# powturbo/Turbo-Range-Coder

Hardware: AMD Instinct MI355X
Metric: encode+decode MB/s, order-0 static-CDF rANS, 100 MB bytes (higher is better)
Workload: dtype u32; 1 GPU; text100m: 100000000 B/GPU, static-CDF rANS, 2 states (anscdf4senc/anscdf4sdec per chunk), tables in LDS, chunk 512 B, 1 lane = 1 chunk, 64 chunks/wave; codec=anscdf4s, chunk=512, bytes_per_gpu=100000000, compressed_bytes_per_gpu=64522350, steps_in_flight=1, exchange=none

## Files before the change

turbo-range-coder_amd/csrc/trc_dir.hip:

```cpp
#include <stdlib.h>
#include "trc_dev.h"
#include "trc_launch.h"

__global__ __launch_bounds__(256) void trc_static_prep_kernel(const u16 *__restrict__ cdf, u32 cdfnum,
                                                              u8 *__restrict__ tables)
{
    __shared__ u32 c[258];
    const u32 tid = threadIdx.x;
    for (u32 i = tid; i < 258; i += 256) c[i] = (i <= cdfnum) ? (u32)cdf[i] : TRC_PROB_ONE;
    __syncthreads();
    const u32 slot = blockIdx.x * 256 + tid;
    u32 x = 0, hi = 256;
    while (x + 1 < hi) { u32 mid = (x + hi) >> 1; if (c[mid] > slot) hi = mid; else x = mid; }
    tables[TRC_TAB_LUT + slot] = (u8)x;
    if (blockIdx.x == 0) {
        const u32 c0 = c[tid], f = c[tid + 1] - c0;
        uint4 e; u32 d;
        if (f == 0) {
            e = make_uint4(0u, 0u, 0xffffffffu, 0u); d = 1u << 16;
        } else if (f == 1) {
            e = make_uint4(0xffffffffu, TRC_PROB_ONE - 1u, 1u << 16, c0 + TRC_PROB_ONE - 1u); d = (1u << 16) | c0;
        } else {
            const u32 l = 32u - (u32)__clz((int)(f - 1));
            const u32 m = (u32)((((u64)1) << (31 + l)) / f) + 1u;
            e = make_uint4(m, (TRC_PROB_ONE - f) | ((l - 1u) << 24), f << 16, c0);
            d = (f << 16) | c0;
        }
        ((uint4 *)(tables + TRC_TAB_ENC))[tid] = e;
        ((u32 *)(tables + TRC_TAB_DEC))[tid] = d;
        for (u32 i = tid; i < 260; i += 256) ((u16 *)(tables + TRC_TAB_CDF))[i] = (u16)((i <= cdfnum) ? cdf[i] : TRC_PROB_ONE);
    }
}

void trc_launch_static_prep(const uint16_t *d_cdf, unsigned cdfnum, uint8_t *tables, hipStream_t s)
{
    hipLaunchKernelGGL(trc_static_prep_kernel, dim3(128), dim3(256), 0, s, d_cdf, (u32)cdfnum, tables);
}

__global__ __launch_bounds__(256) void trc_group_sums_kernel(const u32 *__restrict__ clen, u32 nchunks, u64 n, u32 chunk,
                                                             u32 *__restrict__ gsum)
{
    const u32 c = blockIdx.x * 256 + threadIdx.x;
    const u64 cstart = (u64)c * chunk;
    const u32 len = c < nchunks ? (u32)((n - cstart) < chunk ? (n - cstart) : chunk) : 0u;
    const u32 v = trc_wave_sum(c < nchunks ? trc_min(clen[c], len) : 0u);
    if (trc_lane() == 0 && (c >> 6) < ((nchunks + 63) >> 6)) gsum[c >> 6] = v;
}
void trc_launch_group_sums(const uint32_t *d_clen, uint32_t nchunks, size_t n, uint32_t chunk, uint32_t *gsum, hipStream_t s)
{
    hipLaunchKernelGGL(trc_group_sums_kernel, dim3((nchunks + 255) / 256), dim3(256), 0, s, d_clen, nchunks, (u64)n, chunk, gsum);
}

__global__ __launch_bounds__(1024) void trc_scan_groups_kernel(const u32 *__restrict__ gsum, u32 ngroups,
                                                               u64 *__restrict__ goff, u64 *__restrict__ total)
{
    __shared__ u32 wsum[16];
    __shared__ u64 base_s;
    const u32 tid = threadIdx.x, lane = tid & 63, wid = tid >> 6;
    if (tid == 0) base_s = 0;
    __syncthreads();
    for (u32 t0 = 0; t0 < ngroups; t0 += 1024) {
        const u32 i = t0 + tid;
        const u32 v = i < ngroups ? gsum[i] : 0u;
        const u32 inc = trc_wave_incl_scan(v);
        if (lane == 63) wsum[wid] = inc;
        __syncthreads();
        u32 wbase = 0;
        for (u32 k = 0; k < wid; k++) wbase += wsum[k];
        const u64 base = base_s;
        if (i < ngroups) goff[i] = base + wbase + inc - v;
        __syncthreads();
        if (tid == 1023) base_s = base + wbase + inc;
        __syncthreads();
    }
    if (tid == 0) { goff[ngroups] = base_s; if (total) *total = base_s; }
}
void trc_launch_scan_groups(const uint32_t *gsum, uint32_t ngroups, uint64_t *goff, uint64_t *d_total, hipStream_t s)
{
    TRC_LAUNCH_TIMED(trc_scan_groups_kernel, dim3(1), dim3(1024), 0, s, gsum, ngroups, goff, d_total);
}

__global__ __launch_bounds__(256) void trc_range_dir_kernel(const u32 *__restrict__ clen, u32 nchunks, u64 n, u32 chunk,
                                                            const u64 *__restrict__ goff_full, u32 first, u32 count,
                                                            u32 *__restrict__ gsum_sub, u64 *__restrict__ goff_sub)
{
    const u32 ngroups_sub = (count + 63u) >> 6, end = first + count;
    const u32 j = blockIdx.x * 4u + (threadIdx.x >> 6), lane = trc_lane();
    if (j > ngroups_sub) return;
    const u32 b = trc_min(first + 64u * j, end);
    auto clamped = [&](u32 c) -> u32 {
        const u64 left = n - (u64)c * chunk;
        return trc_min(clen[c], left < chunk ? (u32)left : chunk);
    };
    const u32 below = (b & ~63u) + lane, mine = b + lane;
    const u32 pre = trc_wave_sum(below < b ? clamped(below) : 0u);
    const u32 sum = trc_wave_sum(mine < end ? clamped(mine) : 0u);
    if (lane == 0) {
        goff_sub[j] = goff_full[b >> 6] + pre;
        if (j < ngroups_sub) gsum_sub[j] = sum;
    }
}
void trc_launch_range_dir(const uint32_t *d_clen, uint32_t nchunks, size_t n, uint32_t chunk, const uint64_t *goff_full,
                          uint32_t first, uint32_t count, uint32_t *gsum_sub, uint64_t *goff_sub, hipStream_t s)
{
    const uint32_t waves = (count + 63u) / 64u + 1u;
    hipLaunchKernelGGL(trc_range_dir_kernel, dim3((waves + 3u) / 4u), dim3(256), 0, s, d_clen, nchunks, (u64)n, chunk, goff_full,
                       first, count, gsum_sub, goff_sub);
}

#ifndef TRC_GATHER_VPT
#define TRC_GATHER_VPT 6
#endif
#ifndef TRC_GATHER_ATTR
#define TRC_GATHER_ATTR
#endif
template <int PARTS>
__global__ __launch_bounds__(256) TRC_GATHER_ATTR void trc_gather_kernel(const u8 *__restrict__ in, u64 n, u32 chunk, u32 nchunks,
                                                         const u8 *__restrict__ scratch, u32 stride, int from_end,
                                                         const u8 *__restrict__ scratch2, u32 stride2, const u32 *__restrict__ aux,
                                                         const u32 *__restrict__ clen, const u64 *__restrict__ goff,
                                                         const u32 *__restrict__ gsum, u32 ngroups,
                                                         u8 *__restrict__ payload, u64 *__restrict__ total, u64 *__restrict__ goff_out)
{
    constexpr u32 NP = 64u * PARTS;
    constexpr u32 TPP = 256u / NP;
    constexpr u32 VPT = TRC_GATHER_VPT;
    __shared__ u32 ex_s[NP + 1];
    __shared__ u64 src_s[NP];
    __shared__ u64 base_s;
    const u32 g = blockIdx.x, tid = threadIdx.x, lane = tid & 63u, wid = tid >> 6;
    if (wid == 1 || blockDim.x == 64) {
        const u64 b = trc_group_base(goff, gsum, g);
        if (lane == 0) { base_s = b; if (goff_out) goff_out[g] = b; }
    }
    if (wid == 0) {
        const u32 c = g * 64 + lane;
        const u32 l = c < nchunks ? clen[c] : 0u;
        const u64 cstart = (u64)c * chunk;
        const u32 len = c < nchunks ? (u32)((n - cstart) < chunk ? (n - cstart) : chunk) : 0u;
        const bool raw = l == len;
        const u32 inc = trc_wave_incl_scan(l);
        if (PARTS == 1) {
            ex_s[lane] = inc - l;
            src_s[lane] = (u64)(uintptr_t)(raw ? in + cstart : from_end ? scratch + (u64)(c + 1) * stride - l : scratch + (u64)c * stride);
        } else {
            const u8 *a = scratch + (u64)c * stride;
            const u32 la = (raw || c >= nchunks) ? l : from_end >= 3 ? aux[2 * c] : 4u + *(const u32 *)a;
            ex_s[2 * lane] = inc - l; ex_s[2 * lane + 1] = inc - l + la;
            src_s[2 * lane] = (u64)(uintptr_t)(raw ? in + cstart : from_end == 4 ? scratch + (u64)(c + 1) * stride - la : a);
            src_s[2 * lane + 1] = (u64)(uintptr_t)(from_end == 3 ? scratch + (u64)(c + 1) * stride - (l - la) :
                                                   from_end == 4 ? scratch2 + (u64)(c + 1) * stride2 - (l - la) : scratch2 + (u64)c * stride2);
        }
        if (lane == 63) ex_s[NP] = inc;
    }
    __syncthreads();
    const u64 base = base_s;
    const u32 tot = ex_s[NP];
    if (total && g == ngroups - 1 && tid == 0) *total = base + tot;
    u8 *dst0 = payload + base;
    auto src_of = [&](u32 p) -> const u8 * { return (const u8 *)(uintptr_t)src_s[p]; };

    u32 head = (u32)((16u - ((uintptr_t)dst0 & 15u)) & 15u);
    if (head > tot) head = tot;
    const u32 nvec = (tot - head) >> 4;
    const u32 tail0 = head + (nvec << 4);
    for (u32 b = tid; b < head + (tot - tail0); b += 256) {
        const u32 d = b < head ? b : tail0 + (b - head);
        u32 lo = 0, hi = NP;
        while (lo + 1 < hi) { const u32 mid = (lo + hi) >> 1; if (ex_s[mid] <= d) lo = mid; else hi = mid; }
        dst0[d] = src_of(lo)[d - ex_s[lo]];
    }
    {
        const u32 k = tid / TPP, sub = tid % TPP;
        const u32 e0 = ex_s[k], e1 = ex_s[k + 1];
        const u32 v_lo = e0 <= head ? 0u : (e0 - head + 15u) >> 4;
        u32 v_hi = e1 <= head ? 0u : (e1 - head + 15u) >> 4;
        if (v_hi > nvec) v_hi = nvec;
        const u8 *sa = src_of(k);
        const u8 *sb = k + 1 < NP ? src_of(k + 1) : sa;
        const u32 e2 = ex_s[k + 2 > NP ? NP : k + 2];
        const u32 pl = e1 - e0;
        const bool a16 = pl >= 16u;
        const bool b16 = k + 1 < NP && e2 - e1 >= 16u;
        auto bytewise = [&](u32 dv) {
            u32 kk = k;
            const u8 *p = sa;
            for (u32 q = 0; q < 16; q++) {
                while (dv + q >= ex_s[kk + 1]) { kk++; p = src_of(kk); }
                dst0[dv + q] = p[dv + q - ex_s[kk]];
            }
        };
        if (!a16) {
            if (sub == 0 && v_lo < v_hi) bytewise(head + (v_lo << 4));
            return;
        }
        for (u32 v0 = v_lo + sub; v0 < v_hi; v0 += VPT * TPP) {
            uint4 a[VPT], b[VPT];
            u32 d[VPT];
            bool ok[VPT];
#pragma unroll
            for (int j = 0; j < (int)VPT; j++) {
                const u32 v = v0 + TPP * (u32)j;
                ok[j] = v < v_hi;
                d[j] = head + ((ok[j] ? v : v0) << 4);
                a[j] = make_uint4(0u, 0u, 0u, 0u);
                if (ok[j]) a[j] = trc_ld16_a2_global(sa + trc_min(d[j] - e0, pl - 16u));
                b[j] = a[j];
            }
#pragma unroll
            for (int j = 0; j < (int)VPT; j++)
                if (ok[j] && d[j] + 16u > e1 && b16) b[j] = trc_ld16_a2_global(sb);
#pragma unroll
            for (int j = 0; j < (int)VPT; j++) {
                if (!ok[j]) continue;
                const u32 sp = e1 - d[j];
                if (sp >= 16u) { *(uint4 *)(dst0 + d[j]) = a[j]; continue; }
                if (b16) *(uint4 *)(dst0 + d[j]) = trc_splice16(a[j], b[j], 16u - sp);
                else bytewise(d[j]);
            }
        }
    }
}
void trc_launch_gather(const uint8_t *d_in, size_t n, uint32_t chunk, const TrcWork &w, TrcGather mode,
                       const uint32_t *d_clen, uint8_t *d_payload, uint64_t *d_total, hipStream_t s)
{
    const int from_end = mode;
    if (from_end >= 2)
        TRC_LAUNCH_TIMED((trc_gather_kernel<2>), dim3(w.ngroups), dim3(256), 0, s, d_in, (u64)n, chunk, w.nchunks,
                           w.scratch, w.stride, from_end >= 3 ? from_end : 0, w.scratch2, w.stride2, w.aux, d_clen, w.goff, w.gsum, w.ngroups,
                           d_payload, w.goff ? (u64 *)nullptr : d_total, w.goff ? (u64 *)nullptr : w.goff_area);
    else
        TRC_LAUNCH_TIMED((trc_gather_kernel<1>), dim3(w.ngroups), dim3(256), 0, s, d_in, (u64)n, chunk, w.nchunks,
                           w.scratch, w.stride, from_end, w.scratch2, w.stride2, w.aux, d_clen, w.goff, w.gsum, w.ngroups,
                           d_payload, w.goff ? (u64 *)nullptr : d_total, w.goff ? (u64 *)nullptr : w.goff_area);
}

#define TRC_HIST2_WAVE_LDS (128u * 16u * 4u)
#define TRC_HIST2_WAVES 16u
#define TRC_HIST2_ROUND_VECS 1023u
__global__ __launch_bounds__(1024) void trc_hist2_kernel(const u8 *__restrict__ in, u64 n, u64 *__restrict__ hist, u32 round_vecs)
{
    extern __shared__ __attribute__((aligned(16))) u8 smem[];
    typedef __attribute__((address_space(3))) u32 lds_u32;
    const u32 tid = threadIdx.x, lane = tid & 63u, wv = tid >> 6;
    u32 *mine = (u32 *)(smem + wv * TRC_HIST2_WAVE_LDS);
    u64 *tot = (u64 *)(smem + TRC_HIST2_WAVES * TRC_HIST2_WAVE_LDS);
    const u32 col = trc_lds_addr(mine) + (lane & 15u) * 4u;
    if (tid < 256u) tot[tid] = 0;
    const u64 nvec = n >> 4, stride = (u64)gridDim.x * 1024;
    const uint4 *v = (const uint4 *)in;
    auto count = [&](u32 w) __attribute__((always_inline)) {
#pragma unroll
        for (int k = 0; k < 4; k++) {
            const u32 a = (__builtin_amdgcn_ubfe(w, 8 * k + 1, 7) << 6) + col;
            const u32 inc = __umul24(__builtin_amdgcn_ubfe(w, 8 * k, 1), 0xffffu) + 1u;
            __hip_atomic_fetch_add((lds_u32 *)(uintptr_t)a, inc, __ATOMIC_RELAXED, __HIP_MEMORY_SCOPE_WAVEFRONT);
        }
    };
    auto count4 = [&](const uint4 q) __attribute__((always_inline)) { count(q.x); count(q.y); count(q.z); count(q.w); };
    for (u64 r0 = 0; r0 == 0 || r0 < nvec; r0 += stride * round_vecs) {
        for (u32 r = lane; r < 128u * 16u; r += 64u) mine[r] = 0;
        u64 i = r0 + (u64)blockIdx.x * 1024 + tid;
        u32 left = round_vecs;
        if (left >= 2u && i + stride < nvec) {
            uint4 q0 = v[i], q1 = v[i + stride];
            left -= 2u; i += 2 * stride;
            for (; left >= 2u && i + stride < nvec; left -= 2u, i += 2 * stride) {
                const uint4 n0 = v[i], n1 = v[i + stride];
                count4(q0); count4(q1);
                q0 = n0; q1 = n1;
            }
            count4(q0); count4(q1);
        }
        for (; left && i < nvec; left--, i += stride) count4(v[i]);
        if (r0 == 0 && blockIdx.x == 0 && wv == 0)
            for (u64 t = (nvec << 4) + lane; t < n; t += 64) {
                const u32 b = in[t];
                __hip_atomic_fetch_add((lds_u32 *)(uintptr_t)(col + (b >> 1) * 64u), (b & 1u) ? 0x10000u : 1u, __ATOMIC_RELAXED, __HIP_MEMORY_SCOPE_WAVEFRONT);
            }
        u32 lo0 = 0, hi0 = 0, lo1 = 0, hi1 = 0;
#pragma unroll
        for (u32 c4 = 0; c4 < 4u; c4++) {
            const uint4 a = *(const uint4 *)(mine + lane * 16u + c4 * 4u), b = *(const uint4 *)(mine + (lane + 64u) * 16u + c4 * 4u);
            lo0 += (a.x & 0xffffu) + (a.y & 0xffffu) + (a.z & 0xffffu) + (a.w & 0xffffu); hi0 += (a.x >> 16) + (a.y >> 16) + (a.z >> 16) + (a.w >> 16);
            lo1 += (b.x & 0xffffu) + (b.y & 0xffffu) + (b.z & 0xffffu) + (b.w & 0xffffu); hi1 += (b.x >> 16) + (b.y >> 16) + (b.z >> 16) + (b.w >> 16);
        }
        __syncthreads();
        atomicAdd((unsigned long long *)&tot[2 * lane], (unsigned long long)lo0);
        atomicAdd((unsigned long long *)&tot[2 * lane + 1], (unsigned long long)hi0);
        atomicAdd((unsigned long long *)&tot[2 * (lane + 64)], (unsigned long long)lo1);
        atomicAdd((unsigned long long *)&tot[2 * (lane + 64) + 1], (unsigned long long)hi1);
    }
    __syncthreads();
    if (tid < 256u) {
        const u32 bin = (tid + 37u * blockIdx.x) & 255u;
        if (tot[bin]) atomicAdd((unsigned long long *)&hist[bin], (unsigned long long)tot[bin]);
    }
}
__global__ __launch_bounds__(256) void trc_cdf_build_kernel(const u64 *__restrict__ hist, u64 n, u32 cdfnum,
                                                            u16 *__restrict__ cdf, int *__restrict__ status)
{
    __shared__ u64 f[256];
    __shared__ u32 pre[257];
    __shared__ int bad;
    const u32 tid = threadIdx.x;
    if (tid == 0) bad = 0;
    u64 v = 0;
    if (tid < cdfnum) { v = (hist[tid] << TRC_PROB_BITS) / n; if (!v) v = 1; }
    f[tid] = v;
    __syncthreads();
    if (tid == 0) {
        u64 best = 0, sum = 0; u32 bi = 0;
        for (u32 i = 0; i < cdfnum; i++) { sum += f[i]; if (f[i] > best) { best = f[i]; bi = i; } }
        f[bi] -= sum - TRC_PROB_ONE;
        u32 acc = 0; pre[0] = 0;
        for (u32 i = 0; i < cdfnum; i++) { acc = (acc + (u32)f[i]) & 0xffffu; pre[i + 1] = acc; }
    }
    __syncthreads();
    if (tid < cdfnum && pre[tid] >= pre[tid + 1]) atomicOr(&bad, 1);
    if (tid == 0 && pre[cdfnum] != (TRC_PROB_ONE & 0xffffu)) atomicOr(&bad, 1);
    __syncthreads();
    for (u32 i = tid; i <= cdfnum; i += 256) cdf[i] = (u16)pre[i];
    if (tid == 0) *status = bad ? -1 : (int)(n > 0x7fffffffull ? 0x7fffffffull : n);
}
void trc_launch_hist(const uint8_t *d_in, size_t n, uint64_t *d_hist, hipStream_t s)
{
    (void)hipMemsetAsync(d_hist, 0, 256 * sizeof(uint64_t), s);
    const size_t sm2 = TRC_HIST2_WAVES * TRC_HIST2_WAVE_LDS + 256u * sizeof(u64);
    u64 b2 = ((n >> 4) + 1023) / 1024;
    b2 = b2 < 1 ? 1 : b2 > 256 ? 256 : b2;
    TRC_RAISE_LDS_ONCE(trc_hist2_kernel, sm2);
    static const u32 rv = getenv("TRC_HIST_ROUND_VECS") ? (u32)atoi(getenv("TRC_HIST_ROUND_VECS")) : TRC_HIST2_ROUND_VECS;
    hipLaunchKernelGGL(trc_hist2_kernel, dim3((u32)b2), dim3(1024), sm2, s, d_in, (u64)n, d_hist,
                       rv >= 1u && rv <= TRC_HIST2_ROUND_VECS ? rv : TRC_HIST2_ROUND_VECS);
}
void trc_launch_cdf_build(const uint64_t *d_hist, size_t n_total, uint16_t *d_cdf, unsigned cdfnum, int32_t *d_status, hipStream_t s)
{
    hipLaunchKernelGGL(trc_cdf_build_kernel, dim3(1), dim3(256), 0, s, d_hist, (u64)n_total, (u32)cdfnum, d_cdf, d_status);
}
void trc_launch_cdfini(const uint8_t *d_in, size_t n, uint16_t *d_cdf, unsigned cdfnum,
                       int32_t *d_status, uint64_t *d_hist, hipStream_t s)
{
    trc_launch_hist(d_in, n, d_hist, s);
    trc_launch_cdf_build(d_hist, n, d_cdf, cdfnum, d_status, s);
}
```

Baseline: 729,500 MB/s.

## Restructure gather into 64-byte-aligned sectors with per-piece ownership and edge vectors

Result: faster. 739,300 MB/s (median of 6 runs) (+1.3%).

```diff
diff --git a/turbo-range-coder_amd/csrc/trc_dir.hip b/turbo-range-coder_amd/csrc/trc_dir.hip
--- a/turbo-range-coder_amd/csrc/trc_dir.hip
+++ b/turbo-range-coder_amd/csrc/trc_dir.hip
@@ -114,6 +114,9 @@
 #ifndef TRC_GATHER_ATTR
 #define TRC_GATHER_ATTR
 #endif
+#ifdef TRC_GATHER_PROF
+__device__ unsigned long long trc_gat_wall[16 * 4096];
+#endif
 template <int PARTS>
 __global__ __launch_bounds__(256) TRC_GATHER_ATTR void trc_gather_kernel(const u8 *__restrict__ in, u64 n, u32 chunk, u32 nchunks,
                                                          const u8 *__restrict__ scratch, u32 stride, int from_end,
@@ -129,6 +132,9 @@
     __shared__ u64 src_s[NP];
     __shared__ u64 base_s;
     const u32 g = blockIdx.x, tid = threadIdx.x, lane = tid & 63u, wid = tid >> 6;
+#ifdef TRC_GATHER_PROF
+    const u64 gw0 = wall_clock64();
+#endif
     if (wid == 1 || blockDim.x == 64) {
         const u64 b = trc_group_base(goff, gsum, g);
         if (lane == 0) { base_s = b; if (goff_out) goff_out[g] = b; }
@@ -154,6 +160,9 @@
         if (lane == 63) ex_s[NP] = inc;
     }
     __syncthreads();
+#ifdef TRC_GATHER_PROF
+    const u64 gw1 = wall_clock64();
+#endif
     const u64 base = base_s;
     const u32 tot = ex_s[NP];
     if (total && g == ngroups - 1 && tid == 0) *total = base + tot;
@@ -164,63 +173,116 @@
     if (head > tot) head = tot;
     const u32 nvec = (tot - head) >> 4;
     const u32 tail0 = head + (nvec << 4);
+    const u32 sh = (u32)((64u - ((uintptr_t)dst0 & 63u)) & 63u);
+    const u32 nsec = tot > sh ? (tot - sh) >> 6 : 0u;
+    auto bytewise = [&](u32 dv, u32 kk) {
+        const u8 *p = src_of(kk);
+        for (u32 q = 0; q < 16; q++) {
+            while (dv + q >= ex_s[kk + 1]) { kk++; p = src_of(kk); }
+            dst0[dv + q] = p[dv + q - ex_s[kk]];
+        }
+    };
+    auto piece_of = [&](u32 d) -> u32 {
+        u32 lo = 0, hi = NP;
+        while (lo + 1 < hi) { const u32 mid = (lo + hi) >> 1; if (ex_s[mid] <= d) lo = mid; else hi = mid; }
+        return lo;
+    };
     for (u32 b = tid; b < head + (tot - tail0); b += 256) {
         const u32 d = b < head ? b : tail0 + (b - head);
-        u32 lo = 0, hi = NP;
-        while (lo + 1 < hi) { const u32 mid = (lo + hi) >> 1; if (ex_s[mid] <= d) lo = mid; else hi = mid; }
+        const u32 lo = piece_of(d);
         dst0[d] = src_of(lo)[d - ex_s[lo]];
+    }
+    {
+        const u32 nv1 = ((tot < sh ? tot : sh) - head) >> 4;
+        const u32 nv2 = nvec - nv1 - 4u * nsec;
+        const u32 e = tid - 64u;
+        if (e < nv1 + nv2) {
+            const u32 dv = e < nv1 ? head + (e << 4) : sh + (nsec << 6) + ((e - nv1) << 4);
+            const u32 lo = piece_of(dv);
+            if (dv + 16u <= ex_s[lo + 1]) *(uint4 *)(dst0 + dv) = trc_ld16_a2_global(src_of(lo) + (dv - ex_s[lo]));
+            else bytewise(dv, lo);
+        }
     }
     {
         const u32 k = tid / TPP, sub = tid % TPP;
         const u32 e0 = ex_s[k], e1 = ex_s[k + 1];
-        const u32 v_lo = e0 <= head ? 0u : (e0 - head + 15u) >> 4;
-        u32 v_hi = e1 <= head ? 0u : (e1 - head + 15u) >> 4;
-        if (v_hi > nvec) v_hi = nvec;
-        const u8 *sa = src_of(k);
-        const u8 *sb = k + 1 < NP ? src_of(k + 1) : sa;
-        const u32 e2 = ex_s[k + 2 > NP ? NP : k + 2];
-        const u32 pl = e1 - e0;
-        const bool a16 = pl >= 16u;
-        const bool b16 = k + 1 < NP && e2 - e1 >= 16u;
-        auto bytewise = [&](u32 dv) {
-            u32 kk = k;
-            const u8 *p = sa;
-            for (u32 q = 0; q < 16; q++) {
-                while (dv + q >= ex_s[kk + 1]) { kk++; p = src_of(kk); }
-                dst0[dv + q] = p[dv + q - ex_s[kk]];
+        const u32 s_lo = e0 <= sh ? 0u : (e0 - sh + 63u) >> 6;
+        u32 s_hi = e1 <= sh ? 0u : (e1 - sh + 63u) >> 6;
+        if (s_hi > nsec) s_hi = nsec;
+        if (s_lo < s_hi) {
+            const u8 *sa = src_of(k);
+            const u8 *sb = k + 1 < NP ? src_of(k + 1) : sa;
+            const u32 e2 = ex_s[k + 2 > NP ? NP : k + 2];
+            const u32 pl = e1 - e0;
+            const bool a16 = pl >= 16u;
+            const bool b16 = k + 1 < NP && e2 - e1 >= 16u;
+            constexpr u32 LV = 4u / TPP;
+            enum { WHOLE, SPLICE, BYTES };
+            uint4 la[LV], lb[LV];
+            u32 ld[LV], lk[LV];
+#pragma unroll
+            for (int i = 0; i < (int)LV; i++) {
+                const u32 d = sh + ((4u * (s_hi - 1u) + sub + TPP * (u32)i) << 4);
+                ld[i] = d; lk[i] = BYTES;
+                la[i] = make_uint4(0u, 0u, 0u, 0u); lb[i] = la[i];
+                if (d + 16u <= e1) { la[i] = trc_ld16_a2_global(sa + (d - e0)); lk[i] = WHOLE; }
+                else if (d < e1) { if (a16 && b16) { la[i] = trc_ld16_a2_global(sa + (pl - 16u)); lb[i] = trc_ld16_a2_global(sb); lk[i] = SPLICE; } }
+                else if (d + 16u <= e2) { la[i] = trc_ld16_a2_global(sb + (d - e1)); lk[i] = WHOLE; }
             }
-        };
-        if (!a16) {
-            if (sub == 0 && v_lo < v_hi) bytewise(head + (v_lo << 4));
-            return;
-        }
-        for (u32 v0 = v_lo + sub; v0 < v_hi; v0 += VPT * TPP) {
-            uint4 a[VPT], b[VPT];
-            u32 d[VPT];
-            bool ok[VPT];
-#pragma unroll
-            for (int j = 0; j < (int)VPT; j++) {
-                const u32 v = v0 + TPP * (u32)j;
-                ok[j] = v < v_hi;
-                d[j] = head + ((ok[j] ? v : v0) << 4);
-                a[j] = make_uint4(0u, 0u, 0u, 0u);
-                if (ok[j]) a[j] = trc_ld16_a2_global(sa + trc_min(d[j] - e0, pl - 16u));
-                b[j] = a[j];
+            const u32 u_hi = 4u * (s_hi - 1u);
+            for (u32 u0 = 4u * s_lo + sub; u0 < u_hi; u0 += VPT * TPP) {
+                uint4 a[VPT];
+#pragma unroll
+                for (int j = 0; j < (int)VPT; j++) {
+                    const u32 u = u0 + TPP * (u32)j;
+                    if (u < u_hi) a[j] = trc_ld16_a2_global(sa + (sh + (u << 4) - e0));
+                }
+#pragma unroll
+                for (int j = 0; j < (int)VPT; j++) {
+                    const u32 u = u0 + TPP * (u32)j;
+                    if (u < u_hi) *(uint4 *)(dst0 + sh + (u << 4)) = a[j];
+                }
             }
 #pragma unroll
-            for (int j = 0; j < (int)VPT; j++)
-                if (ok[j] && d[j] + 16u > e1 && b16) b[j] = trc_ld16_a2_global(sb);
-#pragma unroll
-            for (int j = 0; j < (int)VPT; j++) {
-                if (!ok[j]) continue;
-                const u32 sp = e1 - d[j];
-                if (sp >= 16u) { *(uint4 *)(dst0 + d[j]) = a[j]; continue; }
-                if (b16) *(uint4 *)(dst0 + d[j]) = trc_splice16(a[j], b[j], 16u - sp);
-                else bytewise(d[j]);
+            for (int i = 0; i < (int)LV; i++) {
+                if (lk[i] == WHOLE) *(uint4 *)(dst0 + ld[i]) = la[i];
+                else if (lk[i] == SPLICE) *(uint4 *)(dst0 + ld[i]) = trc_splice16(la[i], lb[i], 16u - (e1 - ld[i]));
+                else bytewise(ld[i], k);
             }
         }
     }
-}
+#ifdef TRC_GATHER_PROF
+    {
+        const u64 gw2 = wall_clock64();
+        asm volatile("s_waitcnt vmcnt(0)" ::: "memory");
+        const u64 gw3 = wall_clock64();
+        if (lane == 0) { unsigned long long *w = trc_gat_wall + 16u * (g & 4095u) + 4u * (wid & 3u); w[0] = gw0; w[1] = gw1; w[2] = gw2; w[3] = gw3; }
+    }
+#endif
+}
+#ifdef TRC_GATHER_PROF
+#include <stdio.h>
+static void trc_gather_prof_report(u32 ngroups)
+{
+    static int calls = 0;
+    if (++calls % 64 != 0) return;
+    static unsigned long long wl[16 * 4096];
+    (void)hipDeviceSynchronize();
+    (void)hipMemcpyFromSymbol(wl, HIP_SYMBOL(trc_gat_wall), sizeof wl);
+    const unsigned ng = ngroups < 4096u ? ngroups : 4096u;
+    unsigned long long t0 = ~0ull;
+    for (unsigned i = 0; i < 16 * ng; i += 4) if (wl[i] && wl[i] < t0) t0 = wl[i];
+    double first_ready = 1e9, last_start = 0, sum_ready = 0, last_issue = 0, last_ack = 0, sum_ack = 0; unsigned cnt = 0;
+    for (unsigned i = 0; i < 16 * ng; i += 4) {
+        if (!wl[i]) continue;
+        const double a = (wl[i] - t0) * 0.01, b = (wl[i + 1] - t0) * 0.01, c = (wl[i + 2] - t0) * 0.01, d = (wl[i + 3] - t0) * 0.01;
+        if (a > last_start) last_start = a; if (b < first_ready) first_ready = b; if (c > last_issue) last_issue = c; if (d > last_ack) last_ack = d;
+        sum_ready += b - a; sum_ack += d - a; cnt++;
+    }
+    fprintf(stderr, "[gather wall, us since the first wave's start] waves %u, last start %.2f; first table ready %.2f (mean %.2f after a wave's own start); last store issued %.2f, last store acknowledged %.2f (mean wave life %.2f)\n",
+            cnt, last_start, first_ready, cnt ? sum_ready / cnt : 0.0, last_issue, last_ack, cnt ? sum_ack / cnt : 0.0);
+}
+#endif
 void trc_launch_gather(const uint8_t *d_in, size_t n, uint32_t chunk, const TrcWork &w, TrcGather mode,
                        const uint32_t *d_clen, uint8_t *d_payload, uint64_t *d_total, hipStream_t s)
 {
@@ -233,6 +295,9 @@
         TRC_LAUNCH_TIMED((trc_gather_kernel<1>), dim3(w.ngroups), dim3(256), 0, s, d_in, (u64)n, chunk, w.nchunks,
                            w.scratch, w.stride, from_end, w.scratch2, w.stride2, w.aux, d_clen, w.goff, w.gsum, w.ngroups,
                            d_payload, w.goff ? (u64 *)nullptr : d_total, w.goff ? (u64 *)nullptr : w.goff_area);
+#ifdef TRC_GATHER_PROF
+    trc_gather_prof_report(w.ngroups);
+#endif
 }
 
 #define TRC_HIST2_WAVE_LDS (128u * 16u * 4u)
```
